# rdspring1/lightning-thunder

Measured on AMD Instinct MI355X. Metric: tokens/sec/GPU Llama-2-7B pretrain (LitGPT) + speedup vs eager at 1/2/4/8 MI355X, higher is better.
Workload: dtype bf16; 1 GPU; model=Llama-2-7b-hf, global_batch=1, micro_batch=1, seq_len=4096, parallelism=single, mode=thunder, optimizer=AdamW

## Files before the change

lightning_thunder_amd/ops/attention.py:

```python
from __future__ import annotations

import ctypes
import math
import os

import torch

from ._lib import require, dcode, ptr, stream_ptr, check, register_signature, c_int, c_int64, c_void_p, c_float

register_signature("lta_attn_fwd", [c_int, c_void_p, c_void_p, c_void_p, c_void_p, c_void_p, c_int, c_int, c_int, c_int,
                                    c_int, c_int, c_float, c_int, c_void_p])
register_signature("lta_attn_bwd", [c_int, c_void_p, c_void_p, c_void_p, c_void_p, c_void_p, c_void_p, c_void_p,
                                    c_void_p, c_void_p, c_void_p, c_void_p, c_int, c_int, c_int, c_int, c_int, c_int,
                                    c_float, c_int, c_void_p])
register_signature("lta_attn_fwd_s", [c_int, c_void_p, c_void_p, c_void_p, c_void_p, c_void_p, c_int, c_int, c_int,
                                      c_int, c_int, c_int, c_float, c_int, c_void_p, c_void_p])
register_signature("lta_attn_bwd_s", [c_int, c_void_p, c_void_p, c_void_p, c_void_p, c_void_p, c_void_p, c_void_p,
                                      c_void_p, c_void_p, c_void_p, c_void_p, c_int, c_int, c_int, c_int, c_int, c_int,
                                      c_float, c_int, c_void_p, c_void_p])

register_signature("lta_attn_fwd_ex", [c_int, c_void_p, c_void_p, c_void_p, c_void_p, c_void_p, c_int, c_int, c_int,
                                       c_int, c_int, c_int, c_float, c_int, c_void_p, c_void_p, c_int, c_int, c_float,
                                       ctypes.c_uint64, ctypes.c_uint64, c_void_p])
register_signature("lta_attn_bwd_ex", [c_int, c_void_p, c_void_p, c_void_p, c_void_p, c_void_p, c_void_p, c_void_p,
                                       c_void_p, c_void_p, c_void_p, c_int, c_int, c_int, c_int, c_int, c_int, c_float,
                                       c_int, c_void_p, c_void_p, c_int, c_int, c_void_p, c_float, ctypes.c_uint64,
                                       ctypes.c_uint64, c_void_p])

register_signature("lta_attn_fwd_ex2", [c_int, c_void_p, c_void_p, c_void_p, c_void_p, c_void_p, c_int, c_int, c_int,
                                        c_int, c_int, c_int, c_float, c_int, c_void_p, c_void_p, c_int, c_int, c_float,
                                        ctypes.c_uint64, ctypes.c_uint64, c_void_p, c_void_p])
register_signature("lta_attn_bwd_ex2", [c_int, c_void_p, c_void_p, c_void_p, c_void_p, c_void_p, c_void_p, c_void_p,
                                        c_void_p, c_void_p, c_void_p, c_int, c_int, c_int, c_int, c_int, c_int, c_float,
                                        c_int, c_void_p, c_void_p, c_int, c_int, c_void_p, c_float, ctypes.c_uint64,
                                        ctypes.c_uint64, c_void_p, c_void_p])
register_signature("lta_attn_bwd_rope", [c_int, c_void_p, c_void_p, c_void_p, c_void_p, c_void_p, c_void_p, c_void_p,
                                         c_void_p, c_void_p, c_void_p, c_int, c_int, c_int, c_int, c_int, c_int, c_float,
                                         c_int, c_void_p, c_void_p, c_void_p, c_void_p, c_void_p, c_void_p,
                                         ctypes.c_int64, c_int, c_void_p])
register_signature("lta_attn_bwd_rope_ds", [c_int, c_void_p, c_void_p, c_void_p, c_void_p, c_void_p, c_void_p,
                                            c_void_p, c_void_p, c_void_p, c_void_p, c_int, c_int, c_int, c_int, c_int,
                                            c_int, c_float, c_int, c_void_p, c_void_p, c_void_p, c_void_p, c_void_p,
                                            c_void_p, ctypes.c_int64, c_void_p, ctypes.c_int64, c_int, c_void_p])
register_signature("lta_attn_bwd_ex3", [c_int, c_void_p, c_void_p, c_void_p, c_void_p, c_void_p, c_void_p, c_void_p,
                                        c_void_p, c_void_p, c_void_p, c_int, c_int, c_int, c_int, c_int, c_int, c_float,
                                        c_int, c_void_p, c_void_p, c_int, c_int, c_void_p, c_float, ctypes.c_uint64,
                                        ctypes.c_uint64, c_void_p, c_void_p, c_void_p])

SUPPORTED_HEAD_DIMS = (64, 96, 128, 256)
MAX_PADDED_HEAD_DIM = 256
PLAIN_ONLY_HEAD_DIM = 256


def padded_head_dim(D: int) -> int | None:
    if D in SUPPORTED_HEAD_DIMS:
        return D
    if D % 8 or D <= 0 or D > MAX_PADDED_HEAD_DIM:
        return None
    return next(d for d in SUPPORTED_HEAD_DIMS if d >= D)


def _pad_d(t: torch.Tensor, Dp: int) -> torch.Tensor:
    return t if t.shape[-1] == Dp else torch.nn.functional.pad(t, (0, Dp - t.shape[-1]))


def prepare_mask(mask: torch.Tensor, B: int, Hq: int, Tq: int, Sk: int):
    m = mask
    while m.dim() < 4:
        m = m.unsqueeze(0)
    mb = m.shape[0] == B and B > 1
    mh = m.shape[1] == Hq and Hq > 1
    m = m.expand(B if mb else 1, Hq if mh else 1, Tq, Sk)
    skp = (Sk + 63) // 64 * 64
    out = torch.full((m.shape[0], m.shape[1], Tq, skp), float("-inf"), device=m.device, dtype=torch.float32)
    if m.dtype == torch.bool:
        out[..., :Sk].masked_fill_(m, 0.0)
    else:
        out[..., :Sk].copy_(m)
    return out, int(mb), int(mh)


def supported(q, k, v) -> bool:
    return (
        q.dtype in (torch.bfloat16, torch.float16)
        and k.dtype == q.dtype
        and v.dtype == q.dtype
        and q.ndim == 4
        and padded_head_dim(q.shape[-1]) is not None
        and k.shape[-1] == q.shape[-1]
        and v.shape[-1] == q.shape[-1]
        and q.shape[1] % k.shape[1] == 0
        and k.shape[1] == v.shape[1]
    )


def _c(t):
    return t if t.is_contiguous() else t.contiguous()


def _strides3(t):
    return (ctypes.c_int64 * 3)(*t.stride()[:3])


def _qkv_in_place(q, k, v):
    q, k, v = (_rows_in_place(t) for t in (q, k, v))
    st = (ctypes.c_int64 * 9)(*q.stride()[:3], *k.stride()[:3], *v.stride()[:3])
    return q, k, v, st


def _grad_like(t):
    B, H, T, D = t.shape
    if H > 1 and T > 1 and t.stride(2) > t.stride(1):
        return torch.empty((B, T, H, D), device=t.device, dtype=t.dtype).transpose(1, 2)
    return torch.empty((B, H, T, D), device=t.device, dtype=t.dtype)


def _rows_ok(t) -> bool:
    return t.stride(-1) == 1 and all(s % 8 == 0 for s in t.stride()[:-1]) and t.data_ptr() % 16 == 0


def _rows_in_place(t):
    if _rows_ok(t):
        return t
    return t.clone(memory_format=torch.contiguous_format) if t.is_contiguous() else t.contiguous()


register_signature("lta_attn_set_rng_state", [c_void_p])
register_signature("lta_attn_set_fp8_out", [c_void_p, c_void_p, c_float, c_void_p, c_void_p])
register_signature("lta_attn_fp8_out_used", [])

# ... 350 lines not shown
```

lightning_thunder_amd/ops/csrc/attention_bwd.hip:

```cpp
#include "attention.h"

using namespace lta;
using namespace lta::attn;

namespace {

constexpr int kThreads = 256;
typedef __attribute__((address_space(3))) void lds_void;
typedef float f32x4v __attribute__((ext_vector_type(4)));

template <int D> struct BCfg {
  static constexpr int BN = D > 128 ? 32 : 64;
  static constexpr int NKT = BN / 32;
  static constexpr int RSTR = D + 8;
  static constexpr int TSTR = D + 32;
  static constexpr int CH = D / 8;
  static constexpr int KS = D / 16;
  static constexpr int DT = D / 32;
};

struct RowStrides {
  int64_t b, h, t;
};

// ... 683 lines not shown
          }
        }
        stamp(it, 4);
        tr_wait16(xt, xr);
#pragma unroll
        for (int dt = 0; dt < C::DT; ++dt)
#pragma unroll
          for (int j = 0; j < 2; ++j) {
            mfma_acc_agpr(dkacc[j][dt], xt[2 * dt], df[j][0]);
            mfma_acc_agpr(dkacc[j][dt], xt[2 * dt + 1], df[j][1]);
          }
        if constexpr (WDS) {
          const int hq_cur = hbase + it / nq;
          const int nqb = (Tq + 255) >> 8;
          const uint64_t wa = (uint64_t)(uintptr_t)(dSt + ((((int64_t)(b * Hq + hq_cur) * nqb + (qbase >> 8)) * Sk + kw) * 256 +
                                                           (qbase & 255)));
          const uint64_t wu = ((uint64_t)(uint32_t)__builtin_amdgcn_readfirstlane((int)(wa >> 32)) << 32) |
                              (uint32_t)__builtin_amdgcn_readfirstlane((int)(uint32_t)wa);
          const int wbytes = __builtin_amdgcn_readfirstlane(max(0, min(64, Sk - kw)) * 512);
          const __amdgpu_buffer_rsrc_t rs =
              __builtin_amdgcn_make_buffer_rsrc((void*)(uintptr_t)wu, (short)0, wbytes, 0x00020000);
          const int loff = (r * 256 + 8 * h) * 2;
#pragma unroll
          for (int j = 0; j < 2; ++j) {
            __builtin_amdgcn_raw_buffer_store_b128(__builtin_bit_cast(dsi32x4, df[j][0]), rs, loff, j * 16384, 2);
            __builtin_amdgcn_raw_buffer_store_b128(__builtin_bit_cast(dsi32x4, df[j][1]), rs, loff, j * 16384 + 32, 2);
          }
        }
      }
    }
    stamp(it, 5);
    if (issue_next) {
      advance();
      wait_all_but_newest(true);
      stash_stats(st2);
    } else {
      asm volatile("s_waitcnt vmcnt(0)" ::: "memory");
    }
    stamp(it, 6);
    asm volatile("s_waitcnt lgkmcnt(0)" ::: "memory");
    __builtin_amdgcn_s_barrier();
    asm volatile("" ::: "memory");
    stamp(it, 7);
    ti = ti + 1 == nq ? 0 : ti + 1;
    st = st == 2 ? 0 : st + 1;
  }
  if constexpr (STAMP != 0) {
    if (blockIdx.x == 0 && blockIdx.y == 0 && dbg != nullptr) {
      __syncthreads();
      for (int i = tid; i < 4 * 64 * 8; i += kThreads) dbg[i] = *reinterpret_cast<const uint64_t*>(smem + SBASE + i * 8);
    }
  }
#pragma unroll
  for (int j = 0; j < 2; ++j)
#pragma unroll
    for (int dt = 0; dt < C::DT; ++dt) asm volatile("s_nop 15\n\ts_nop 15" : "+a"(dkacc[j][dt]), "+a"(dvacc[j][dt]));

  if constexpr (SPLIT) {
#pragma unroll
    for (int j = 0; j < 2; ++j) {
      const int key = kw + 32 * j + r;
      if (key < Sk) {
        const int64_t nbh = gridDim.x / nsplit;
        float* prow = part + (((int64_t)hs * nbh + bh) * Sk + key) * 256;
        const bool rope = sx.rope_cos != nullptr;
        store_row_d128_f32(prow, dkacc[j], scale, h, rope ? sx.rope_cos + (int64_t)key * 128 : nullptr,
                           rope ? sx.rope_sin + (int64_t)key * 128 : nullptr);
        store_row_d128_f32(prow + 128, dvacc[j], 1.f, h, nullptr, nullptr);
      }
    }
    return;
  }
#pragma unroll
  for (int j = 0; j < 2; ++j) {
    const int key = kw + 32 * j + r;
    if (key < Sk) {
      T* dkrow = dK + (int64_t)b * sx.dkb + (int64_t)hk * sx.dkh + (int64_t)key * sx.dkt;
      T* dvrow = dV + (int64_t)b * sx.dvb + (int64_t)hk * sx.dvh + (int64_t)key * sx.dvt;
      const bool rope = sx.rope_cos != nullptr;
      store_row_d128(dkrow, dkacc[j], scale, h, rope ? sx.rope_cos + (int64_t)key * 128 : nullptr,
                     rope ? sx.rope_sin + (int64_t)key * 128 : nullptr);
      store_row_d128(dvrow, dvacc[j], 1.f, h, nullptr, nullptr);
    }
  }
}

constexpr int kBM = 128;
constexpr int kBN = 64;

template <typename T, int D, bool CAUSAL, int EX = 0>
__global__ __launch_bounds__(kThreads, (EX || D > 128) ? 1 : 2) void attn_bwd_dq_kernel(const T* __restrict__ Q, const T* __restrict__ K,
                                                                  const T* __restrict__ V, const T* __restrict__ dO,
                                                                  const float* __restrict__ LSE,
                                                                  const float* __restrict__ DELTA, T* __restrict__ dQ,
                                                                  int Hq, int Hkv, int Tq, int Sk, float scale,
                                                                  float scale_log2, RowStrides sdo, AttnExtra ex) {
  constexpr bool MASK = EX & kExMask, DROP = EX & kExDrop;
  using C = BCfg<D>;
  using F = typename Frag<T>::type;
  __shared__ __attribute__((aligned(16))) short smem[2 * C::BN * C::RSTR + C::BN * C::TSTR];
  __shared__ __attribute__((aligned(16))) unsigned ktab[DROP ? 4 * C::BN : 4];
  short* Kr = smem;
  short* Vr = Kr + C::BN * C::RSTR;
  short* Kt = Vr + C::BN * C::RSTR;
  const __attribute__((address_space(3))) short* Kt3 = (const __attribute__((address_space(3))) short*)Kt;

  const int n_qt = (Tq + kBM - 1) / kBM;
  const int qt = n_qt - 1 - (int)blockIdx.y;
  const int bh = blockIdx.x;
  const int b = bh / Hq, hq = bh % Hq;
  const int hk = hq / (Hq / Hkv);
  const T* Qb = Q + b * ex.sx.qb + hq * ex.sx.qh;
  const T* dOb = dO + b * sdo.b + hq * sdo.h;
  const T* Kb = K + b * ex.sx.kb + hk * ex.sx.kh;
  const T* Vb = V + b * ex.sx.vb + hk * ex.sx.vh;

  const int tid = threadIdx.x, lane = tid & 63;
  const int wave = __builtin_amdgcn_readfirstlane(tid >> 6);
  const int r = lane & 31, h = lane >> 5, g = lane >> 4, l16 = lane & 15;
  const int q0 = qt * kBM + wave * 32;
  const int qi = q0 + r;
  const int qrow = min(qi, Tq - 1);

  F qf[C::KS], of[C::KS];
#pragma unroll
  for (int s = 0; s < C::KS; ++s) {
    qf[s] = load_frag<F>(Qb + (int64_t)qrow * ex.sx.qt + 16 * s + 8 * h);
    of[s] = load_frag<F>(dOb + qrow * sdo.t + 16 * s + 8 * h);
  }
  float lse2 = LSE[((int64_t)b * Hq + hq) * Tq + qrow] * 1.44269504088896340736f;
  if constexpr (MASK) lse2 = (lse2 == -INFINITY) ? INFINITY : lse2;
  const float dlt = DELTA[((int64_t)b * Hq + hq) * Tq + qrow];
  const float* mrow = nullptr;
  if constexpr (MASK) mrow = ex.mask + b * ex.mb + hq * ex.mh + (int64_t)qrow * ex.mq;
  unsigned qterm = 0;
  if constexpr (DROP) qterm = rng_q(rng_head(ex, bh), qi);

  f32x16 dqacc[C::DT];
#pragma unroll
  for (int dt = 0; dt < C::DT; ++dt)
#pragma unroll
    for (int i = 0; i < 16; ++i) dqacc[dt][i] = 0.f;

  int n_tiles = (Sk + C::BN - 1) / C::BN;
  if (CAUSAL) n_tiles = min(n_tiles, (min(qt * kBM + kBM, Tq) + C::BN - 1) / C::BN);
  constexpr int LOADS = C::BN * C::CH / kThreads;
  static_assert(C::BN * C::CH % kThreads == 0, "K/V staging must cover the tile");

  uint4 pk[LOADS], pv[LOADS];
  auto issue = [&](int t) {
#pragma unroll
    for (int c = 0; c < LOADS; ++c) {
      const int id = c * kThreads + tid;
      const int row = id / C::CH, ch = id % C::CH;
      const int kc = min(t * C::BN + row, Sk - 1);
      pk[c] = *reinterpret_cast<const uint4*>(Kb + (int64_t)kc * ex.sx.kt + ch * 8);
      pv[c] = *reinterpret_cast<const uint4*>(Vb + (int64_t)kc * ex.sx.vt + ch * 8);
    }
  };
  if (n_tiles > 0) issue(0);
  for (int t = 0; t < n_tiles; ++t) {
    __syncthreads();
#pragma unroll
    for (int c = 0; c < LOADS; ++c) {
      const int id = c * kThreads + tid;
      const int row = id / C::CH, ch = id % C::CH;
// ... 425 lines not shown
#pragma unroll
  for (int blk = 0; blk < 4; ++blk)
    koff[blk] = (4 * hh + vq) * 256 + ((4 * (blk ^ vq) + 2 * (g & 1) + (vp >> 1)) << 4) + 8 * (vp & 1);
#pragma unroll
  for (int x = 0; x < 2; ++x)
    soff[x] = (4 * hh + vq) * 512 + ((4 * ((2 * wave + x) ^ vq) + 2 * (g & 1) + (vp >> 1)) << 4) + 8 * (vp & 1);

  f32x16 acc[2][4];
#pragma unroll
  for (int x = 0; x < 2; ++x)
#pragma unroll
    for (int dt = 0; dt < 4; ++dt)
#pragma unroll
      for (int i = 0; i < 16; ++i) acc[x][dt][i] = 0.f;

#pragma unroll
  for (int p = 0; p < NST - 1; ++p)
    if (p < nt) issue(p, p);
  for (int t = 0; t < nt; ++t) {
    static_assert(NST == 3, "one tile in flight behind the one waited for");
    if (t + 1 < nt)
      asm volatile("s_waitcnt vmcnt(%0)" ::"n"(NK + NS) : "memory");
    else
      asm volatile("s_waitcnt vmcnt(0)" ::: "memory");
    __builtin_amdgcn_s_barrier();
    if (t + NST - 1 < nt) issue(t + NST - 1, (t + NST - 1) % NST);
    const uint32_t kimg = lds0 + (t % NST) * STG, simg = kimg + KIMG;
    const uint32_t ka[4] = {kimg + koff[0], kimg + koff[1], kimg + koff[2], kimg + koff[3]};
    const uint32_t sa[2] = {simg + soff[0], simg + soff[1]};
    s16x4t xa[12], xb[12];
    dqds_issue<0>(xa, ka, sa);
    dqds_steps<0, KT / 16, F>(acc, xa, xb, ka, sa);
  }
#pragma unroll
  for (int x = 0; x < 2; ++x)
#pragma unroll
    for (int dt = 0; dt < 4; ++dt) asm volatile("s_nop 15\n\ts_nop 15" : "+a"(acc[x][dt]));
  const bool rope = sx.rope_cos != nullptr;
#pragma unroll
  for (int x = 0; x < 2; ++x) {
    const int n = lane & 31, e = n & 7;
    const int q = q0 + 32 * (2 * wave + x) + (e & 3) + 8 * (e >> 2) + 4 * ((n >> 3) & 1) + 16 * (n >> 4);
    if (q < Tq) {
      T* qrow = dQ + (int64_t)b * sx.dqb + (int64_t)hq * sx.dqh + (int64_t)q * sx.dqt;
      store_row_d128(qrow, acc[x], scale, hh, rope ? sx.rope_cos + (int64_t)q * 128 : nullptr,
                     rope ? sx.rope_sin + (int64_t)q * 128 : nullptr);
    }
  }
}


template <typename T, int D, int EX>
void launch_masked(const void* dO, const void* Q, const void* K, const void* V, const void* LSE, void* DELTA, void* dQ,
                   void* dK, void* dV, int B, int Hq, int Hkv, int Tq, int Sk, float scale, float sl2, int causal,
                   RowStrides sdo, const AttnExtra& ex, hipStream_t s) {
  dim3 g1(B * Hkv, (Sk + kKB - 1) / kKB), g2(B * Hq, (Tq + kBM - 1) / kBM), blk(kThreads);
  constexpr int EXQ = EX & (kExMask | kExDrop);
#define LTA_DKDV(CA)                                                                                               \
  hipLaunchKernelGGL((attn_bwd_dkdv_kernel<T, D, CA, EX>), g1, blk, 0, s, (const T*)Q, (const T*)K, (const T*)V,   \
                     (const T*)dO, (const float*)LSE, (const float*)DELTA, (T*)dK, (T*)dV, Hq, Hkv, Tq, Sk, scale, sl2, \
                     sdo, ex)
#define LTA_DQ(CA)                                                                                                 \
  hipLaunchKernelGGL((attn_bwd_dq_kernel<T, D, CA, EXQ>), g2, blk, 0, s, (const T*)Q, (const T*)K, (const T*)V,    \
                     (const T*)dO, (const float*)LSE, (const float*)DELTA, (T*)dQ, Hq, Hkv, Tq, Sk, scale, sl2, sdo, ex)
  if (causal) {
    LTA_DKDV(true);
    LTA_DQ(true);
  } else {
    LTA_DKDV(false);
    LTA_DQ(false);
  }
#undef LTA_DKDV
#undef LTA_DQ
}

#ifdef LTA_ATTN_DIAG
uint64_t* g_dkdv_stamps = nullptr;
#endif
int g_dkdv_qrev = [] {
  const char* e = getenv("LTA_DKDV_QREV");
  return (e && e[0] == '0') ? 0 : 1;
}();

#ifdef LTA_ATTN_DIAG
#define LTA_DKDV_LAUNCH(CA)                                                                                          \
  if (g_dkdv_stamps)                                                                                                 \
    hipLaunchKernelGGL((attn_bwd_dkdv_v4_kernel<T, CA, 1>), gk, blk, 0, s, (const T*)Q, (const T*)K, (const T*)V,   \
                       (const T*)dO, (const float*)LSE, (const float*)DELTA, (T*)dK, (T*)dV, Hq, Hkv, Tq, Sk, scale, \
                       sl2, sdo, ex.sx, g_dkdv_qrev, g_dkdv_stamps);                                                  \
  else                                                                                                               \
    hipLaunchKernelGGL((attn_bwd_dkdv_v4_kernel<T, CA>), gk, blk, 0, s, (const T*)Q, (const T*)K, (const T*)V,       \
                       (const T*)dO, (const float*)LSE, (const float*)DELTA, (T*)dK, (T*)dV, Hq, Hkv, Tq, Sk, scale, \
                       sl2, sdo, ex.sx, g_dkdv_qrev, nullptr)
#else
#define LTA_DKDV_LAUNCH(CA)                                                                                          \
  {                                                                                                                  \
    const int hsplit = (ex.part && ex.hsplit > 1) ? ex.hsplit : 1;                                                   \
    dim3 gks(gk.x * hsplit, gk.y);                                                                                   \
    if (hsplit > 1) {                                                                                                \
      hipLaunchKernelGGL((attn_bwd_dkdv_v4_kernel<T, CA, 0, false, true>), gks, blk, 0, s, (const T*)Q, (const T*)K, \
                         (const T*)V, (const T*)dO, (const float*)LSE, (const float*)DELTA, (T*)dK, (T*)dV, Hq, Hkv,   \
                         Tq, Sk, scale, sl2, sdo, ex.sx, g_dkdv_qrev, nullptr, nullptr, hsplit, ex.part);            \
      launch_dkdv_reduce<T>(dK, dV, B, Hkv, Sk, ex, s);                                                              \
    } else {                                                                                                         \
      hipLaunchKernelGGL((attn_bwd_dkdv_v4_kernel<T, CA>), gk, blk, 0, s, (const T*)Q, (const T*)K, (const T*)V,     \
                         (const T*)dO, (const float*)LSE, (const float*)DELTA, (T*)dK, (T*)dV, Hq, Hkv, Tq, Sk,       \
                         scale, sl2, sdo, ex.sx, g_dkdv_qrev, nullptr);                                              \
    }                                                                                                                \
  }
#endif

template <typename T, int D = 128>
__global__ __launch_bounds__(256) void attn_bwd_dkdv_reduce(const float* __restrict__ part, T* __restrict__ dK,
                                                            T* __restrict__ dV, int nbh, int Hkv, int Sk, int hsplit,
                                                            QKVStrides sx) {
  constexpr int CH = D / 8;
  const int64_t id = (int64_t)blockIdx.x * 256 + threadIdx.x;
  if (id >= (int64_t)nbh * Sk * 2 * CH) return;
  const int c = (int)(id % CH);
  const int64_t row = id / CH;
  const int which = (int)(row & 1);
  const int64_t bk = row >> 1;
  const int key = (int)(bk % Sk), bh = (int)(bk / Sk);
  float acc[8] = {0.f, 0.f, 0.f, 0.f, 0.f, 0.f, 0.f, 0.f};
  for (int s = 0; s < hsplit; ++s) {
    const float4* src = reinterpret_cast<const float4*>(part + (((int64_t)s * nbh + bh) * Sk + key) * (2 * D) + which * D + c * 8);
    const float4 a = src[0], b = src[1];
    acc[0] += a.x; acc[1] += a.y; acc[2] += a.z; acc[3] += a.w;
    acc[4] += b.x; acc[5] += b.y; acc[6] += b.z; acc[7] += b.w;
  }
  const int b = bh / Hkv, hk = bh % Hkv;
  T* dst = which ? dV + (int64_t)b * sx.dvb + (int64_t)hk * sx.dvh + (int64_t)key * sx.dvt
                 : dK + (int64_t)b * sx.dkb + (int64_t)hk * sx.dkh + (int64_t)key * sx.dkt;
  union {
    T v[8];
    uint4 u;
  } pk;
#pragma unroll
  for (int e = 0; e < 8; ++e) pk.v[e] = from_f32<T>(acc[e]);
  *reinterpret_cast<uint4*>(dst + c * 8) = pk.u;
}

template <typename T, int D = 128>
void launch_dkdv_reduce(void* dK, void* dV, int B, int Hkv, int Sk, const AttnExtra& ex, hipStream_t s) {
  const int64_t n = (int64_t)B * Hkv * Sk * 2 * (D / 8);
  hipLaunchKernelGGL((attn_bwd_dkdv_reduce<T, D>), dim3((unsigned)((n + 255) / 256)), dim3(256), 0, s,
                     (const float*)ex.part, (T*)dK, (T*)dV, B * Hkv, Hkv, Sk, ex.hsplit, ex.sx);
}

template <typename T>
int launch_bwd_ds(const void* dO, const void* Q, const void* K, const void* V, const void* O, const void* LSE,
                  void* DELTA, void* dQ, void* dK, void* dV, void* dS, int B, int Hq, int Hkv, int Tq, int Sk,
                  float scale, int causal, RowStrides sdo, RowStrides so, const AttnExtra& ex, hipStream_t s) {
  const float sl2 = scale * 1.44269504088896340736f;
  const int64_t rows = (int64_t)B * Hq * Tq;
  dim3 blk(kThreads);
  hipLaunchKernelGGL((attn_bwd_preprocess<T, 128>), dim3((unsigned)((rows * 8 + 255) / 256)), dim3(256), 0, s,
                     (const T*)dO, (const T*)O, (float*)DELTA, rows, Hq, Tq, sdo, so);
  const int hsplit = (ex.part && ex.hsplit > 1) ? ex.hsplit : 1;
  dim3 gk(B * Hkv * hsplit, (Sk + kKB3 - 1) / kKB3), gq(B * Hq, (Tq + 255) / 256);
#define LTA_DS(CA)                                                                                                   \
  if (hsplit > 1) {                                                                                                  \
    hipLaunchKernelGGL((attn_bwd_dkdv_v4_kernel<T, CA, 0, true, true>), gk, blk, 0, s, (const T*)Q, (const T*)K,   \
                       (const T*)V, (const T*)dO, (const float*)LSE, (const float*)DELTA, (T*)dK, (T*)dV, Hq, Hkv, Tq,  \
                       Sk, scale, sl2, sdo, ex.sx, g_dkdv_qrev, nullptr, (T*)dS, hsplit, ex.part);                   \
    launch_dkdv_reduce<T>(dK, dV, B, Hkv, Sk, ex, s);                                                                \
  } else {                                                                                                           \
    hipLaunchKernelGGL((attn_bwd_dkdv_v4_kernel<T, CA, 0, true>), gk, blk, 0, s, (const T*)Q, (const T*)K,          \
                       (const T*)V, (const T*)dO, (const float*)LSE, (const float*)DELTA, (T*)dK, (T*)dV, Hq, Hkv, Tq,  \
                       Sk, scale, sl2, sdo, ex.sx, g_dkdv_qrev, nullptr, (T*)dS);                                    \
  }                                                                                                                  \
  hipLaunchKernelGGL((attn_bwd_dq_ds_kernel<T, CA>), gq, blk, 0, s, (const T*)K, (const T*)dS, (T*)dQ, Hq, Hkv, Tq,   \
                     Sk, scale, ex.sx)
  if (causal) { LTA_DS(true); }
  else { LTA_DS(false); }
#undef LTA_DS
  return (int)hipGetLastError();
}

template <typename T, int D>
int launch_bwd(const void* dO, const void* Q, const void* K, const void* V, const void* O, const void* LSE, void* DELTA,
               void* dQ, void* dK, void* dV, int B, int Hq, int Hkv, int Tq, int Sk, float scale, int causal,
               RowStrides sdo, RowStrides so, int fast, const AttnExtra& ex, int exf, hipStream_t s) {
  const float sl2 = scale * 1.44269504088896340736f;
  const int64_t rows = (int64_t)B * Hq * Tq;
  dim3 blk(kThreads);
  if (exf == 0 && D == 128 && fast && Tq > 0 && Sk > 0) {
    dim3 gq(B * Hq, (Tq + kQB3 - 1) / kQB3), gk(B * Hkv, (Sk + kKB3 - 1) / kKB3);
#define LTA_FAST(CA)                                                                                                 \
  hipLaunchKernelGGL((attn_bwd_dq_v4_kernel<T, CA>), gq, blk, 0, s, (const T*)Q, (const T*)K, (const T*)V,            \
                     (const T*)dO, (const float*)LSE, (const float*)DELTA, (T*)dQ, Hq, Hkv, Tq, Sk, scale, sl2, sdo,   \
                     ex.sx, (const T*)O, so);                                                                          \
  LTA_DKDV_LAUNCH(CA)
    if (causal) { LTA_FAST(true); }
    else { LTA_FAST(false); }
#undef LTA_FAST
    return (int)hipGetLastError();
  }
  hipLaunchKernelGGL((attn_bwd_preprocess<T, D>), dim3((unsigned)((rows * 8 + 255) / 256)), dim3(256), 0, s,
                     (const T*)dO, (const T*)O, (float*)DELTA, rows, Hq, Tq, sdo, so);
  if (exf) {
    switch (exf) {
#define LTA_M(F)                                                                                                  \
  case F:                                                                                                         \
    launch_masked<T, D, F>(dO, Q, K, V, LSE, DELTA, dQ, dK, dV, B, Hq, Hkv, Tq, Sk, scale, sl2, causal, sdo, ex, s); \
    break;
      LTA_M(kExMask)
      LTA_M(kExDrop)
      LTA_M(kExMask | kExDrop)
      LTA_M(kExMask | kExMaskGrad)
      LTA_M(kExMask | kExDrop | kExMaskGrad)
#undef LTA_M
      default:
        return -1;
    }
    return (int)hipGetLastError();
  }
  const int hsplit = (ex.part && ex.hsplit > 1) ? ex.hsplit : 1;
  dim3 g1(B * Hkv * hsplit, (Sk + kKB - 1) / kKB), g2(B * Hq, (Tq + kBM - 1) / kBM);
#define LTA_V1(CA)                                                                                                   \
  if (hsplit > 1) {                                                                                                  \
    hipLaunchKernelGGL((attn_bwd_dkdv_kernel<T, D, CA, 0, true>), g1, blk, 0, s, (const T*)Q, (const T*)K,           \
                       (const T*)V, (const T*)dO, (const float*)LSE, (const float*)DELTA, (T*)dK, (T*)dV, Hq, Hkv, Tq, \
                       Sk, scale, sl2, sdo, ex);                                                                       \
    launch_dkdv_reduce<T, D>(dK, dV, B, Hkv, Sk, ex, s);                                                               \
  } else {                                                                                                           \
    hipLaunchKernelGGL((attn_bwd_dkdv_kernel<T, D, CA>), g1, blk, 0, s, (const T*)Q, (const T*)K, (const T*)V,        \
                       (const T*)dO, (const float*)LSE, (const float*)DELTA, (T*)dK, (T*)dV, Hq, Hkv, Tq, Sk, scale,   \
                       sl2, sdo, ex);                                                                                  \
  }                                                                                                                  \
  hipLaunchKernelGGL((attn_bwd_dq_kernel<T, D, CA>), g2, blk, 0, s, (const T*)Q, (const T*)K, (const T*)V,            \
                     (const T*)dO, (const float*)LSE, (const float*)DELTA, (T*)dQ, Hq, Hkv, Tq, Sk, scale, sl2, sdo, ex)
  if (causal) { LTA_V1(true); }
  else { LTA_V1(false); }
#undef LTA_V1
  return (int)hipGetLastError();
}

}

static int fast_enabled() {
  static const int fast = [] {
    const char* e = getenv("LTA_ATTN_BWD_V1");
    return (e && e[0] == '1') ? 0 : 1;
  }();
  return fast;
}

static bool gqa_split_ok(AttnExtra& ex, void* part_ws, int64_t part_bytes, int hsplit, int B, int Hq, int Hkv, int Sk,
                         int D = 128) {
  if (hsplit <= 1 || part_ws == nullptr) return true;
  const int group = Hq / Hkv;
  if (group % hsplit != 0 || part_bytes < (int64_t)hsplit * B * Hkv * Sk * 2 * D * 4 || (uintptr_t)part_ws % 16) return false;
// ... 84 lines not shown
  if (mask) {
    const int64_t skp = (int64_t)(Sk + 63) / 64 * 64;
    ex.mask = (const float*)mask;
    ex.mq = skp;
    ex.mh = mask_h ? (int64_t)Tq * skp : 0;
    ex.mb = mask_b ? (int64_t)(mask_h ? Hq : 1) * Tq * skp : 0;
    exf |= kExMask;
    if (dmask) {
      ex.dmask = (float*)dmask;
      exf |= kExMaskGrad;
    }
  }
  if (dropout_p > 0.f) {
    ex.keep_scale = 1.f / (1.f - dropout_p);
    ex.keep_thresh = (unsigned)fmin((double)dropout_p * 4294967296.0, 4294967295.0);
    ex.seed_lo = (unsigned)seed;
    ex.seed_hi = (unsigned)(seed >> 32);
    ex.offset = (unsigned)offset;
    ex.rng = rng;
    exf |= kExDrop;
  }
#define LTA_B(TT, DD)                                                                                             \
  return launch_bwd<TT, DD>(dO, Q, K, V, O, LSE, DELTA, dQ, dK, dV, B, Hq, Hkv, Tq, Sk, scale, causal, sdo, so, v2, ex, \
                            exf, stream)
  if (dtype == kBF16) {
    if (D == 128) LTA_B(__hip_bfloat16, 128);
    if (D == 64) LTA_B(__hip_bfloat16, 64);
    if (D == 96) LTA_B(__hip_bfloat16, 96);
    if (D == 256) LTA_B(__hip_bfloat16, 256);
  } else if (dtype == kF16) {
    if (D == 128) LTA_B(__half, 128);
    if (D == 64) LTA_B(__half, 64);
    if (D == 96) LTA_B(__half, 96);
    if (D == 256) LTA_B(__half, 256);
  }
#undef LTA_B
  return -1;
}

LTA_EXPORT int lta_attn_bwd_ex2(int dtype, const void* dO, const void* Q, const void* K, const void* V, const void* O,
                                const void* LSE, void* DELTA, void* dQ, void* dK, void* dV, int B, int Hq, int Hkv,
                                int Tq, int Sk, int D, float scale, int causal, const int64_t* strides, const void* mask,
                                int mask_b, int mask_h, void* dmask, float dropout_p, uint64_t seed, uint64_t offset,
                                const int64_t* qkv_strides, hipStream_t stream) {
  return lta_attn_bwd_ex3(dtype, dO, Q, K, V, O, LSE, DELTA, dQ, dK, dV, B, Hq, Hkv, Tq, Sk, D, scale, causal, strides,
                          mask, mask_b, mask_h, dmask, dropout_p, seed, offset, qkv_strides, nullptr, stream);
}

LTA_EXPORT int lta_attn_bwd_ex(int dtype, const void* dO, const void* Q, const void* K, const void* V, const void* O,
                               const void* LSE, void* DELTA, void* dQ, void* dK, void* dV, int B, int Hq, int Hkv,
                               int Tq, int Sk, int D, float scale, int causal, const int64_t* strides, const void* mask,
                               int mask_b, int mask_h, void* dmask, float dropout_p, uint64_t seed, uint64_t offset,
                               hipStream_t stream) {
  return lta_attn_bwd_ex2(dtype, dO, Q, K, V, O, LSE, DELTA, dQ, dK, dV, B, Hq, Hkv, Tq, Sk, D, scale, causal, strides,
                          mask, mask_b, mask_h, dmask, dropout_p, seed, offset, nullptr, stream);
}

LTA_EXPORT int lta_attn_bwd_s(int dtype, const void* dO, const void* Q, const void* K, const void* V, const void* O,
                              const void* LSE, void* DELTA, void* dQ, void* dK, void* dV, void* workspace, int B, int Hq,
                              int Hkv, int Tq, int Sk, int D, float scale, int causal, const int64_t* strides,
                              hipStream_t stream) {
  return lta_attn_bwd_ex(dtype, dO, Q, K, V, O, LSE, DELTA, dQ, dK, dV, B, Hq, Hkv, Tq, Sk, D, scale, causal, strides,
                         nullptr, 0, 0, nullptr, 0.f, 0, 0, stream);
}

LTA_EXPORT int lta_attn_bwd(int dtype, const void* dO, const void* Q, const void* K, const void* V, const void* O,
                            const void* LSE, void* DELTA, void* dQ, void* dK, void* dV, void* workspace, int B, int Hq,
                            int Hkv, int Tq, int Sk, int D, float scale, int causal, hipStream_t stream) {
  return lta_attn_bwd_s(dtype, dO, Q, K, V, O, LSE, DELTA, dQ, dK, dV, workspace, B, Hq, Hkv, Tq, Sk, D, scale, causal,
                        nullptr, stream);
}

#ifdef LTA_ATTN_DIAG
LTA_EXPORT int lta_attn_bwd_set_stamps(void* dbg) {
  g_dkdv_stamps = (uint64_t*)dbg;
  return 0;
}
#endif
LTA_EXPORT int lta_attn_bwd_set_dkdv_qrev(int rev) {
  const int old = g_dkdv_qrev;
  g_dkdv_qrev = rev ? 1 : 0;
  return old;
}
```

Baseline: 24930 tokens/s.

## Add 512-thread triple-buffered dK/dV attention backward kernel with LDS transpose reads

```diff
diff --git a/lightning_thunder_amd/ops/attention.py b/lightning_thunder_amd/ops/attention.py
--- a/lightning_thunder_amd/ops/attention.py
+++ b/lightning_thunder_amd/ops/attention.py
@@ -46,6 +46,8 @@
                                         c_void_p, c_void_p, c_void_p, c_int, c_int, c_int, c_int, c_int, c_int, c_float,
                                         c_int, c_void_p, c_void_p, c_int, c_int, c_void_p, c_float, ctypes.c_uint64,
                                         ctypes.c_uint64, c_void_p, c_void_p, c_void_p])
+register_signature("lta_attn_bwd_set_dkdv_impl", [c_int])
+register_signature("lta_attn_bwd_last_dkdv_impl", [])
 
 SUPPORTED_HEAD_DIMS = (64, 96, 128, 256)
 MAX_PADDED_HEAD_DIM = 256
diff --git a/lightning_thunder_amd/ops/csrc/attention_bwd.hip b/lightning_thunder_amd/ops/csrc/attention_bwd.hip
--- a/lightning_thunder_amd/ops/csrc/attention_bwd.hip
+++ b/lightning_thunder_amd/ops/csrc/attention_bwd.hip
@@ -789,6 +789,333 @@
                      rope ? sx.rope_sin + (int64_t)key * 128 : nullptr);
       store_row_d128(dvrow, dvacc[j], 1.f, h, nullptr, nullptr);
     }
+  }
+}
+
+constexpr int kThreads5 = 512;
+
+__device__ __forceinline__ void tr_issue8(s16x4t (&x)[8], unsigned ba, unsigned bb) {
+  asm volatile(
+      "ds_read_b64_tr_b16 %0, %8\n\tds_read_b64_tr_b16 %1, %9\n\t"
+      "ds_read_b64_tr_b16 %2, %8 offset:4096\n\tds_read_b64_tr_b16 %3, %9 offset:4096\n\t"
+      "ds_read_b64_tr_b16 %4, %8 offset:512\n\tds_read_b64_tr_b16 %5, %9 offset:512\n\t"
+      "ds_read_b64_tr_b16 %6, %8 offset:4608\n\tds_read_b64_tr_b16 %7, %9 offset:4608"
+      : "=&v"(x[0]), "=&v"(x[1]), "=&v"(x[2]), "=&v"(x[3]), "=&v"(x[4]), "=&v"(x[5]), "=&v"(x[6]), "=&v"(x[7])
+      : "v"(ba), "v"(bb)
+      : "memory");
+}
+template <int N, typename F>
+__device__ __forceinline__ void tr_wait8(F (&f)[4], s16x4t (&x)[8]) {
+  static_assert(N == 0 || N == 8 || N == 16, "groups are 8 reads");
+  if constexpr (N == 16)
+    asm volatile("s_waitcnt lgkmcnt(15)"
+                 : "+v"(x[0]), "+v"(x[1]), "+v"(x[2]), "+v"(x[3]), "+v"(x[4]), "+v"(x[5]), "+v"(x[6]), "+v"(x[7])
+                 :
+                 : "memory");
+  else if constexpr (N == 8)
+    asm volatile("s_waitcnt lgkmcnt(8)"
+                 : "+v"(x[0]), "+v"(x[1]), "+v"(x[2]), "+v"(x[3]), "+v"(x[4]), "+v"(x[5]), "+v"(x[6]), "+v"(x[7])
+                 :
+                 : "memory");
+  else
+    asm volatile("s_waitcnt lgkmcnt(0)"
+                 : "+v"(x[0]), "+v"(x[1]), "+v"(x[2]), "+v"(x[3]), "+v"(x[4]), "+v"(x[5]), "+v"(x[6]), "+v"(x[7])
+                 :
+                 : "memory");
+#pragma unroll
+  for (int i = 0; i < 4; ++i) {
+    union {
+      struct { s16x4t a, b; } s;
+      F f;
+    } u;
+    u.s.a = x[2 * i];
+    u.s.b = x[2 * i + 1];
+    f[i] = u.f;
+  }
+}
+
+template <typename T, bool CAUSAL, bool WDS = false, bool SPLIT = false>
+__global__ __launch_bounds__(kThreads5, 1) void attn_bwd_dkdv_v5_kernel(
+    const T* __restrict__ Q, const T* __restrict__ K, const T* __restrict__ V, const T* __restrict__ dO,
+    const float* __restrict__ LSE, const float* __restrict__ DELTA, T* __restrict__ dK, T* __restrict__ dV, int Hq,
+    int Hkv, int Tq, int Sk, float scale, float scale_log2, RowStrides sdo, QKVStrides sx, int qrev,
+    T* __restrict__ dSt, int hsplit, float* __restrict__ part) {
+  constexpr int D = 128;
+  using C = BCfg<D>;
+  using F = typename Frag<T>::type;
+  constexpr int NST = 3;
+  constexpr int IMG = kQT * 256;
+  constexpr int STAGE = 2 * IMG + 256;
+  constexpr int VOFF = NST * STAGE;
+  constexpr int SBASE = VOFF + kKB3 * C::RSTR * 2;
+  __shared__ __attribute__((aligned(1024))) char smem[SBASE];
+  short* Vs = reinterpret_cast<short*>(smem + VOFF);
+
+  const int kb = (int)blockIdx.y;
+  const int nsplit = SPLIT ? hsplit : 1;
+  const int bh = SPLIT ? (int)blockIdx.x / nsplit : (int)blockIdx.x, hs = SPLIT ? (int)blockIdx.x % nsplit : 0;
+  const int b = bh / Hkv, hk = bh % Hkv;
+  const int group = Hq / Hkv;
+  const int gsz = group / nsplit, hbase = hk * group + hs * gsz;
+  const int tid = threadIdx.x, lane = tid & 63;
+  const int wave = __builtin_amdgcn_readfirstlane(tid >> 6);
+  const int r = lane & 31, h = lane >> 5;
+  const int kw = kb * kKB3 + wave * 32;
+  const T* Kb = K + b * sx.kb + hk * sx.kh;
+  const T* Vb = V + b * sx.vb + hk * sx.vh;
+
+#pragma unroll
+  for (int c = 0; c < kKB3 * C::CH / kThreads5; ++c) {
+    const int id = c * kThreads5 + tid;
+    const int row = id / C::CH, ch = id % C::CH;
+    const int vr = min(kb * kKB3 + row, Sk - 1);
+    *reinterpret_cast<uint4*>(Vs + row * C::RSTR + ch * 8) = *reinterpret_cast<const uint4*>(Vb + (int64_t)vr * sx.vt + ch * 8);
+  }
+  F kf[C::KS];
+  {
+    const int kr = min(kw + r, Sk - 1);
+#pragma unroll
+    for (int s = 0; s < C::KS; ++s) kf[s] = load_frag<F>(Kb + (int64_t)kr * sx.kt + 16 * s + 8 * h);
+  }
+
+  f32x16 dkacc[C::DT], dvacc[C::DT];
+#pragma unroll
+  for (int dt = 0; dt < C::DT; ++dt)
+#pragma unroll
+    for (int i = 0; i < 16; ++i) {
+      dkacc[dt][i] = 0.f;
+      dvacc[dt][i] = 0.f;
+    }
+
+  const int n_qt = (Tq + kQT - 1) / kQT;
+  const int qt_begin = CAUSAL ? min((kb * kKB3) / kQT, n_qt) : 0;
+  const int nq = n_qt - qt_begin;
+  const int total = gsz * nq;
+
+  float plse = 0.f, pdel = 0.f;
+  auto stash_stats = [&](int st) {
+    if (wave == 0 && lane < kQT) {
+      float* sp = reinterpret_cast<float*>(smem + st * STAGE + 2 * IMG);
+      sp[lane] = -plse * 1.44269504088896340736f;
+      sp[kQT + lane] = pdel;
+    }
+  };
+  auto issue = [&](int hi, int ti, int st) {
+    const int hq = hbase + hi;
+    const int qbase = (qt_begin + (qrev ? nq - 1 - ti : ti)) * kQT;
+    const T* Qb = Q + b * sx.qb + hq * sx.qh;
+    const T* dOb = dO + b * sdo.b + hq * sdo.h;
+    char* qimg = smem + st * STAGE;
+    if (wave == 0) {
+      const int64_t srow = ((int64_t)b * Hq + hq) * Tq + min(qbase + (lane & 31), Tq - 1);
+      asm volatile("global_load_dword %0, %2, off\n\tglobal_load_dword %1, %3, off"
+                   : "=&v"(plse), "=&v"(pdel)
+                   : "v"(LSE + srow), "v"(DELTA + srow)
+                   : "memory");
+    }
+    const int u = 64 * wave + lane;
+    const int row = ((u >> 7) << 3) | ((u >> 2) & 7);
+    const int ch = (((u >> 5) & 3) << 2) | ((u & 3) ^ ((row >> 2) & 3));
+    const int qc = min(qbase + row, Tq - 1);
+    __builtin_amdgcn_global_load_lds((const void*)(Qb + (int64_t)qc * sx.qt + ch * 8), (lds_void*)(qimg + wave * 1024), 16,
+                                     0, 0);
+    __builtin_amdgcn_global_load_lds((const void*)(dOb + qc * sdo.t + ch * 8), (lds_void*)(qimg + IMG + wave * 1024), 16,
+                                     0, 0);
+  };
+  auto wait_all_but_newest = [&](bool after_stores) {
+    if (WDS && after_stores)
+      asm volatile("s_waitcnt vmcnt(4)" : "+v"(plse), "+v"(pdel)::"memory");
+    else
+      asm volatile("s_waitcnt vmcnt(2)" : "+v"(plse), "+v"(pdel)::"memory");
+  };
+
+  int nhi = 0, nti = 0;
+  auto advance = [&]() {
+    if (++nti == nq) {
+      nti = 0;
+      ++nhi;
+    }
+  };
+  asm volatile("s_waitcnt vmcnt(0)" ::: "memory");
+  if (total > 0) {
+    issue(nhi, nti, 0);
+    advance();
+    asm volatile("s_waitcnt vmcnt(0)" : "+v"(plse), "+v"(pdel)::"memory");
+    stash_stats(0);
+  }
+  if (total > 1) {
+    issue(nhi, nti, 1);
+    advance();
+    wait_all_but_newest(false);
+    stash_stats(1);
+  }
+  __syncthreads();
+  if (wave >= 4) __builtin_amdgcn_s_setprio(1);
+
+  int ti = 0, st = 0;
+  for (int it = 0; it < total; ++it) {
+    const bool issue_next = it + 2 < total;
+    const int st2 = st >= 1 ? st - 1 : 2;
+    if (issue_next) issue(nhi, nti, st2);
+    const int qt_abs = qt_begin + (qrev ? nq - 1 - ti : ti);
+    const int qbase = qt_abs * kQT;
+    {
+      const char* qimg = smem + st * STAGE;
+      const char* oimg = qimg + IMG;
+      const float* sl = reinterpret_cast<const float*>(qimg + 2 * IMG);
+      unsigned tr_a, tr_b;
+      {
+        const int l16 = lane & 15, g = lane >> 4;
+        const int q = l16 >> 2, p = l16 & 3, cl = 2 * (g & 1) + (p >> 1);
+        const unsigned base = (unsigned)(uintptr_t)(__attribute__((address_space(3))) char*)smem + (unsigned)(st * STAGE);
+        tr_a = base + 64 * (4 * h + q) + 16 * (cl ^ h) + 8 * (p & 1);
+        tr_b = base + 2048 + 64 * (4 * h + q) + 16 * (cl ^ (2 + h)) + 8 * (p & 1);
+      }
+      f32x4v L[4];
+#pragma unroll
+      for (int a = 0; a < 4; ++a) L[a] = *reinterpret_cast<const f32x4v*>(sl + 4 * h + 8 * a);
+      f32x16 sacc, pacc;
+      F pf[2], df[2];
+#pragma unroll
+      for (int i = 0; i < 16; ++i) {
+        sacc[i] = 0.f;
+        pacc[i] = 0.f;
+      }
+      {
+        F qa[C::KS];
+#pragma unroll
+        for (int s = 0; s < 4; ++s) qa[s] = load_frag<F>(qimg + du_off(r, 2 * s + h));
+#pragma unroll
+        for (int s = 0; s < C::KS; ++s) {
+          if (s + 4 < C::KS) qa[s + 4] = load_frag<F>(qimg + du_off(r, 2 * (s + 4) + h));
+          sacc = mfma(qa[s], kf[s], sacc);
+        }
+      }
+      __builtin_amdgcn_sched_barrier(0);
+      {
+        F oa = load_frag<F>(oimg + du_off(r, h));
+        F va = load_frag<F>(Vs + (wave * 32 + r) * C::RSTR + 8 * h);
+#pragma unroll
+        for (int s = 0; s < C::KS; ++s) {
+          F ob = oa, vb = va;
+          if (s + 1 < C::KS) {
+            ob = load_frag<F>(oimg + du_off(r, 2 * (s + 1) + h));
+            vb = load_frag<F>(Vs + (wave * 32 + r) * C::RSTR + 16 * (s + 1) + 8 * h);
+          }
+          pacc = mfma(oa, va, pacc);
+#pragma unroll
+          for (int i = 2 * s; i < 2 * s + 2; ++i)
+            sacc[i] = __builtin_amdgcn_exp2f(__builtin_fmaf(sacc[i], scale_log2, L[i >> 2][i & 3]));
+          if (s == 5) pack_frag(pf[0], sacc, 0);
+          __builtin_amdgcn_sched_barrier(0);
+          oa = ob;
+          va = vb;
+        }
+      }
+      f32x4v Dl[4];
+#pragma unroll
+      for (int a = 0; a < 2; ++a) Dl[a] = *reinterpret_cast<const f32x4v*>(sl + kQT + 4 * h + 8 * a);
+      s16x4t x0[8], x1[8], x2[8];
+      tr_issue8(x0, tr_a + (unsigned)IMG, tr_b + (unsigned)IMG);
+      {
+        const int key = kw + r;
+        const bool masked = (CAUSAL && kw + 31 > qbase) || kw + 32 > Sk || qbase + kQT > Tq;
+        if (masked) {
+#pragma unroll
+          for (int i = 0; i < 16; ++i) {
+            const int qq = qbase + acc_row(i, h);
+            if (key >= Sk || qq >= Tq || (CAUSAL && key > qq)) sacc[i] = 0.f;
+          }
+          pack_frag(pf[0], sacc, 0);
+        }
+      }
+      pack_frag(pf[1], sacc, 1);
+#pragma unroll
+      for (int i = 0; i < 8; ++i) pacc[i] = sacc[i] * (pacc[i] - Dl[i >> 2][i & 3]);
+      pack_frag(df[0], pacc, 0);
+      asm volatile("" : "+v"(df[0]));
+#pragma unroll
+      for (int a = 2; a < 4; ++a) Dl[a] = *reinterpret_cast<const f32x4v*>(sl + kQT + 4 * h + 8 * a);
+#pragma unroll
+      for (int i = 8; i < 16; ++i) pacc[i] = sacc[i] * (pacc[i] - Dl[i >> 2][i & 3]);
+      pack_frag(df[1], pacc, 1);
+      __builtin_amdgcn_sched_barrier(0);
+      tr_issue8(x1, tr_a + (unsigned)(IMG + 1024), tr_b + (unsigned)(IMG + 1024));
+      tr_issue8(x2, tr_a, tr_b);
+      {
+        F xt[4];
+        tr_wait8<16>(xt, x0);
+        mfma_acc_agpr(dvacc[0], xt[0], pf[0]);
+        mfma_acc_agpr(dvacc[0], xt[1], pf[1]);
+        mfma_acc_agpr(dvacc[1], xt[2], pf[0]);
+        mfma_acc_agpr(dvacc[1], xt[3], pf[1]);
+        __builtin_amdgcn_sched_barrier(0);
+        tr_issue8(x0, tr_a + 1024u, tr_b + 1024u);
+        tr_wait8<16>(xt, x1);
+        mfma_acc_agpr(dvacc[2], xt[0], pf[0]);
+        mfma_acc_agpr(dvacc[2], xt[1], pf[1]);
+        mfma_acc_agpr(dvacc[3], xt[2], pf[0]);
+        mfma_acc_agpr(dvacc[3], xt[3], pf[1]);
+        __builtin_amdgcn_sched_barrier(0);
+        tr_wait8<8>(xt, x2);
+        mfma_acc_agpr(dkacc[0], xt[0], df[0]);
+        mfma_acc_agpr(dkacc[0], xt[1], df[1]);
+        mfma_acc_agpr(dkacc[1], xt[2], df[0]);
+        mfma_acc_agpr(dkacc[1], xt[3], df[1]);
+        __builtin_amdgcn_sched_barrier(0);
+        tr_wait8<0>(xt, x0);
+        mfma_acc_agpr(dkacc[2], xt[0], df[0]);
+        mfma_acc_agpr(dkacc[2], xt[1], df[1]);
+        mfma_acc_agpr(dkacc[3], xt[2], df[0]);
+        mfma_acc_agpr(dkacc[3], xt[3], df[1]);
+        if constexpr (WDS) {
+          const int hq_cur = hbase + it / nq;
+          const int nqb = (Tq + 255) >> 8;
+          const uint64_t wa = (uint64_t)(uintptr_t)(dSt + ((((int64_t)(b * Hq + hq_cur) * nqb + (qbase >> 8)) * Sk + kw) * 256 +
+                                                           (qbase & 255)));
+          const uint64_t wu = ((uint64_t)(uint32_t)__builtin_amdgcn_readfirstlane((int)(wa >> 32)) << 32) |
+                              (uint32_t)__builtin_amdgcn_readfirstlane((int)(uint32_t)wa);
+          const int wbytes = __builtin_amdgcn_readfirstlane(max(0, min(32, Sk - kw)) * 512);
+          const __amdgpu_buffer_rsrc_t rs =
+              __builtin_amdgcn_make_buffer_rsrc((void*)(uintptr_t)wu, (short)0, wbytes, 0x00020000);
+          const int loff = (r * 256 + 8 * h) * 2;
+          __builtin_amdgcn_raw_buffer_store_b128(__builtin_bit_cast(dsi32x4, df[0]), rs, loff, 0, 2);
+          __builtin_amdgcn_raw_buffer_store_b128(__builtin_bit_cast(dsi32x4, df[1]), rs, loff, 32, 2);
+        }
+      }
+    }
+    if (issue_next) {
+      advance();
+      wait_all_but_newest(true);
+      stash_stats(st2);
+    } else {
+      asm volatile("s_waitcnt vmcnt(0)" ::: "memory");
+    }
+    asm volatile("s_waitcnt lgkmcnt(0)" ::: "memory");
+    __builtin_amdgcn_s_barrier();
+    asm volatile("" ::: "memory");
+    ti = ti + 1 == nq ? 0 : ti + 1;
+    st = st == 2 ? 0 : st + 1;
+  }
+  if (wave >= 4) __builtin_amdgcn_s_setprio(0);
+#pragma unroll
+  for (int dt = 0; dt < C::DT; ++dt) asm volatile("s_nop 15\n\ts_nop 15" : "+a"(dkacc[dt]), "+a"(dvacc[dt]));
+
+  const int key = kw + r;
+  if (key >= Sk) return;
+  const bool rope = sx.rope_cos != nullptr;
+  if constexpr (SPLIT) {
+    const int64_t nbh = gridDim.x / nsplit;
+    float* prow = part + (((int64_t)hs * nbh + bh) * Sk + key) * 256;
+    store_row_d128_f32(prow, dkacc, scale, h, rope ? sx.rope_cos + (int64_t)key * 128 : nullptr,
+                       rope ? sx.rope_sin + (int64_t)key * 128 : nullptr);
+    store_row_d128_f32(prow + 128, dvacc, 1.f, h, nullptr, nullptr);
+  } else {
+    T* dkrow = dK + (int64_t)b * sx.dkb + (int64_t)hk * sx.dkh + (int64_t)key * sx.dkt;
+    T* dvrow = dV + (int64_t)b * sx.dvb + (int64_t)hk * sx.dvh + (int64_t)key * sx.dvt;
+    store_row_d128(dkrow, dkacc, scale, h, rope ? sx.rope_cos + (int64_t)key * 128 : nullptr,
+                   rope ? sx.rope_sin + (int64_t)key * 128 : nullptr);
+    store_row_d128(dvrow, dvacc, 1.f, h, nullptr, nullptr);
   }
 }
 
@@ -1380,30 +1707,51 @@
   return (e && e[0] == '0') ? 0 : 1;
 }();
 
+constexpr int kDkdvImplDefault = 5;
+int g_dkdv_impl = [] {
+  const char* e = getenv("LTA_ATTN_DKDV");
+  if (e && (e[0] == '4' || e[0] == '5') && e[1] == 0) return e[0] - '0';
+  return kDkdvImplDefault;
+}();
+int g_dkdv_last = 0;
+
+template <typename T, bool CA, bool WDS, bool SPLIT>
+void launch_dkdv_d128(dim3 g, hipStream_t s, const void* Q, const void* K, const void* V, const void* dO,
+                      const void* LSE, const void* DELTA, void* dK, void* dV, int Hq, int Hkv, int Tq, int Sk,
+                      float scale, float sl2, RowStrides sdo, const QKVStrides& sx, void* dS, int hsplit, float* part) {
+  g_dkdv_last = g_dkdv_impl == 5 ? 5 : 4;
+  if (g_dkdv_last == 5)
+    hipLaunchKernelGGL((attn_bwd_dkdv_v5_kernel<T, CA, WDS, SPLIT>), g, dim3(kThreads5), 0, s, (const T*)Q, (const T*)K,
+                       (const T*)V, (const T*)dO, (const float*)LSE, (const float*)DELTA, (T*)dK, (T*)dV, Hq, Hkv, Tq, Sk,
+                       scale, sl2, sdo, sx, g_dkdv_qrev, (T*)dS, hsplit, part);
+  else
+    hipLaunchKernelGGL((attn_bwd_dkdv_v4_kernel<T, CA, 0, WDS, SPLIT>), g, dim3(kThreads), 0, s, (const T*)Q,
+                       (const T*)K, (const T*)V, (const T*)dO, (const float*)LSE, (const float*)DELTA, (T*)dK, (T*)dV, Hq,
+                       Hkv, Tq, Sk, scale, sl2, sdo, sx, g_dkdv_qrev, nullptr, (T*)dS, hsplit, part);
+}
+
 #ifdef LTA_ATTN_DIAG
 #define LTA_DKDV_LAUNCH(CA)                                                                                          \
-  if (g_dkdv_stamps)                                                                                                 \
+  if (g_dkdv_stamps) {                                                                                               \
+    g_dkdv_last = 4;                                                                                                 \
     hipLaunchKernelGGL((attn_bwd_dkdv_v4_kernel<T, CA, 1>), gk, blk, 0, s, (const T*)Q, (const T*)K, (const T*)V,   \
                        (const T*)dO, (const float*)LSE, (const float*)DELTA, (T*)dK, (T*)dV, Hq, Hkv, Tq, Sk, scale, \
                        sl2, sdo, ex.sx, g_dkdv_qrev, g_dkdv_stamps);                                                  \
-  else                                                                                                               \
-    hipLaunchKernelGGL((attn_bwd_dkdv_v4_kernel<T, CA>), gk, blk, 0, s, (const T*)Q, (const T*)K, (const T*)V,       \
-                       (const T*)dO, (const float*)LSE, (const float*)DELTA, (T*)dK, (T*)dV, Hq, Hkv, Tq, Sk, scale, \
-                       sl2, sdo, ex.sx, g_dkdv_qrev, nullptr)
+  } else                                                                                                             \
+    launch_dkdv_d128<T, CA, false, false>(gk, s, Q, K, V, dO, LSE, DELTA, dK, dV, Hq, Hkv, Tq, Sk, scale, sl2, sdo,  \
+                                          ex.sx, nullptr, 1, nullptr)
 #else
 #define LTA_DKDV_LAUNCH(CA)                                                                                          \
   {                                                                                                                  \
     const int hsplit = (ex.part && ex.hsplit > 1) ? ex.hsplit : 1;                                                   \
     dim3 gks(gk.x * hsplit, gk.y);                                                                                   \
     if (hsplit > 1) {                                                                                                \
-      hipLaunchKernelGGL((attn_bwd_dkdv_v4_kernel<T, CA, 0, false, true>), gks, blk, 0, s, (const T*)Q, (const T*)K, \
-                         (const T*)V, (const T*)dO, (const float*)LSE, (const float*)DELTA, (T*)dK, (T*)dV, Hq, Hkv,   \
-                         Tq, Sk, scale, sl2, sdo, ex.sx, g_dkdv_qrev, nullptr, nullptr, hsplit, ex.part);            \
+      launch_dkdv_d128<T, CA, false, true>(gks, s, Q, K, V, dO, LSE, DELTA, dK, dV, Hq, Hkv, Tq, Sk, scale, sl2,     \
+                                           sdo, ex.sx, nullptr, hsplit, ex.part);                                    \
       launch_dkdv_reduce<T>(dK, dV, B, Hkv, Sk, ex, s);                                                              \
     } else {                                                                                                         \
-      hipLaunchKernelGGL((attn_bwd_dkdv_v4_kernel<T, CA>), gk, blk, 0, s, (const T*)Q, (const T*)K, (const T*)V,     \
-                         (const T*)dO, (const float*)LSE, (const float*)DELTA, (T*)dK, (T*)dV, Hq, Hkv, Tq, Sk,       \
-                         scale, sl2, sdo, ex.sx, g_dkdv_qrev, nullptr);                                              \
+      launch_dkdv_d128<T, CA, false, false>(gk, s, Q, K, V, dO, LSE, DELTA, dK, dV, Hq, Hkv, Tq, Sk, scale, sl2,     \
+                                            sdo, ex.sx, nullptr, 1, nullptr);                                        \
     }                                                                                                                \
   }
 #endif
@@ -1459,14 +1807,12 @@
   dim3 gk(B * Hkv * hsplit, (Sk + kKB3 - 1) / kKB3), gq(B * Hq, (Tq + 255) / 256);
 #define LTA_DS(CA)                                                                                                   \
   if (hsplit > 1) {                                                                                                  \
-    hipLaunchKernelGGL((attn_bwd_dkdv_v4_kernel<T, CA, 0, true, true>), gk, blk, 0, s, (const T*)Q, (const T*)K,   \
-                       (const T*)V, (const T*)dO, (const float*)LSE, (const float*)DELTA, (T*)dK, (T*)dV, Hq, Hkv, Tq,  \
-                       Sk, scale, sl2, sdo, ex.sx, g_dkdv_qrev, nullptr, (T*)dS, hsplit, ex.part);                   \
+    launch_dkdv_d128<T, CA, true, true>(gk, s, Q, K, V, dO, LSE, DELTA, dK, dV, Hq, Hkv, Tq, Sk, scale, sl2, sdo,    \
+                                        ex.sx, dS, hsplit, ex.part);                                                 \
     launch_dkdv_reduce<T>(dK, dV, B, Hkv, Sk, ex, s);                                                                \
   } else {                                                                                                           \
-    hipLaunchKernelGGL((attn_bwd_dkdv_v4_kernel<T, CA, 0, true>), gk, blk, 0, s, (const T*)Q, (const T*)K,          \
-                       (const T*)V, (const T*)dO, (const float*)LSE, (const float*)DELTA, (T*)dK, (T*)dV, Hq, Hkv, Tq,  \
-                       Sk, scale, sl2, sdo, ex.sx, g_dkdv_qrev, nullptr, (T*)dS);                                    \
+    launch_dkdv_d128<T, CA, true, false>(gk, s, Q, K, V, dO, LSE, DELTA, dK, dV, Hq, Hkv, Tq, Sk, scale, sl2, sdo,   \
+                                         ex.sx, dS, 1, nullptr);                                                     \
   }                                                                                                                  \
   hipLaunchKernelGGL((attn_bwd_dq_ds_kernel<T, CA>), gq, blk, 0, s, (const T*)K, (const T*)dS, (T*)dQ, Hq, Hkv, Tq,   \
                      Sk, scale, ex.sx)
@@ -1717,3 +2063,11 @@
   g_dkdv_qrev = rev ? 1 : 0;
   return old;
 }
+
+LTA_EXPORT int lta_attn_bwd_set_dkdv_impl(int impl) {
+  const int old = g_dkdv_impl;
+  if (impl == 4 || impl == 5) g_dkdv_impl = impl;
+  return old;
+}
+
+LTA_EXPORT int lta_attn_bwd_last_dkdv_impl() { return g_dkdv_last; }
```

Result: no change. 25100 tokens/s, median of 6 (+0.7%).
